# AuCson/DSP-Speech-Recognition

Measured on AMD Instinct MI355X. Metric: MFCC frames/sec at 16 kHz, 25 ms/10 ms, nfft=512, 40 mel, 13 cep, higher is better.
Workload: dtype f32; 1 GPU; configs[1]: batch of 1024 synthetic 1 s 16 kHz utterances -> MFCC+delta+delta2 [1024*99, 39] per step per GPU; frames_per_utterance=99, delta_n=2, input_buffers_rotated=8, hip_streams=3

## Files before the change

### dsp-speech-recognition_amd/csrc/kernels_fast512.h

```cpp
#pragma once

#include <cmath>
#include <cstdlib>
#include <type_traits>
#include <vector>

#include "dsp_common.h"
#include "launch_common.h"
#include "fft_inreg.h"

#define F512_WAVE_FLOATS 2112
#define F512_PS_STRIDE 264
#define F512_MAX_NI 6
#ifndef F512_WAVES
#define F512_WAVES 8
#endif
#ifndef F512_MIN_WAVES_PER_SIMD
#define F512_MIN_WAVES_PER_SIMD 4
#endif

struct F512Params {
    const float* tables;
    int32_t tab_floats;
    int32_t off_tw1, off_dct, off_melw, off_mels, off_bias, off_coop;
    int32_t melw_row;
    int32_t L, S, M, C, append_energy;
    float preemph;
    int32_t span_vec;
    int32_t nb4[F512_MAX_NI];
    int64_t groups_per_utt, total_groups;
    uint32_t t_magic, t_shift;
    uint32_t g_magic, g_shift;
    int32_t fd_n;
    float fd_inv_den;
    int32_t flat;
    int32_t seam_off;
    const int32_t* group_off;
    const int32_t* group_utt;
};

struct Fast512Plan {
    float* d_tables;
    F512Params P;
    int variant;
    int caps;
};

template <int CTRL>
__device__ __forceinline__ float dpp_f32(float v) {
    return __int_as_float(__builtin_amdgcn_update_dpp(0, __float_as_int(v), CTRL, 0xF, 0xF, true));
}
__device__ __forceinline__ float frame_allreduce(float v) {
    v += dpp_f32<0xB1>(v);
    v += dpp_f32<0x4E>(v);
    v += dpp_f32<0x141>(v);
    return v;
}

__host__ __device__ constexpr int f512_cap(int caps, int i) {
    constexpr int c1[5] = {2, 3, 4, 5, 8}, c2[4] = {3, 4, 6, 12};
    return caps == 1 ? c1[i] : c2[i];
}
__host__ __device__ constexpr int f512_cap_prefix(int caps, int i) {
    int s = 0;
    for (int k = 0; k < i; ++k) s += f512_cap(caps, k);
    return s;
}
template <int I, int N, typename F>
__device__ __forceinline__ void f512_static_for(F&& f) {
    if constexpr (I < N) {
        f(std::integral_constant<int, I>{});
        f512_static_for<I + 1, N>(f);
    }
}
__host__ __device__ constexpr int f512_cbase(int c) { return ((c & 1) ? 2 : 0) ^ ((c & 2) ? 4 : 0) ^ ((c & 4) ? 14 : 0); }
typedef float f512_f2u __attribute__((ext_vector_type(2), aligned(4)));

#define F512_FENCE() asm volatile("" ::: "memory")

#ifdef F512_STAMPS
#define F512_NSTAMP 16
__device__ unsigned int f512_stamp_sum[F512_NSTAMP * 8192];
__device__ __forceinline__ unsigned int f512_clock() {
    unsigned long long t;
    asm volatile("s_waitcnt lgkmcnt(0)\n\ts_memtime %0\n\ts_waitcnt lgkmcnt(0)" : "=s"(t) :: "memory");
    return (unsigned int)t;
}
template <typename T, int N>
__device__ __forceinline__ void f512_pin(T (&a)[N]) {
#pragma unroll
    for (int i = 0; i < N; ++i) {
        if constexpr (sizeof(T) == 8) asm volatile("" : "+v"(a[i].x), "+v"(a[i].y));
        else asm volatile("" : "+v"(a[i]));
    }
}
#ifdef F512_STAMP_ROUNDS
#define F512_STAMP(i)                                                         \
    do {                                                                      \
        if ((i) == 0) stamp_prev_ = f512_clock();                             \
        if ((i) == 10) {                                                      \
            stamp_acc_[r < 4 ? r : 3] += f512_clock() - stamp_prev_;          \
            stamp_acc_[4 + (r < 4 ? r : 3)] += 1;                             \
        }                                                                     \
    } while (0)
#else
#define F512_STAMP(i)                                     \
    do {                                                  \
        const unsigned int now_ = f512_clock();           \
        stamp_acc_[i] += now_ - stamp_prev_;              \
        stamp_prev_ = f512_clock();                       \
    } while (0)
#endif
#define F512_PIN(a) f512_pin(a)
#else
#define F512_STAMP(i) do {} while (0)
#define F512_PIN(a) do {} while (0)
#endif

typedef float f512_v2 __attribute__((ext_vector_type(2)));
__device__ __forceinline__ uint32_t f512_lds_addr(const void* p) {
    return static_cast<uint32_t>(reinterpret_cast<uintptr_t>(p));
}

template <int ROW0>
__device__ __forceinline__ void f512_load_rows8(uint32_t fr, uint32_t wn, f512_v2 (&xv)[8], f512_v2 (&wv)[8]) {
    asm volatile(
        "ds_read_b64 %0, %16 offset:%18\n\tds_read_b64 %8, %17 offset:%18\n\t"
        "ds_read_b64 %1, %16 offset:%19\n\tds_read_b64 %9, %17 offset:%19\n\t"
        "ds_read_b64 %2, %16 offset:%20\n\tds_read_b64 %10, %17 offset:%20\n\t"
        "ds_read_b64 %3, %16 offset:%21\n\tds_read_b64 %11, %17 offset:%21\n\t"
        "ds_read_b64 %4, %16 offset:%22\n\tds_read_b64 %12, %17 offset:%22\n\t"
        "ds_read_b64 %5, %16 offset:%23\n\tds_read_b64 %13, %17 offset:%23\n\t"
        "ds_read_b64 %6, %16 offset:%24\n\tds_read_b64 %14, %17 offset:%24\n\t"
        "ds_read_b64 %7, %16 offset:%25\n\tds_read_b64 %15, %17 offset:%25\n\t"
        "s_waitcnt lgkmcnt(0)"
        : "=&v"(xv[0]), "=&v"(xv[1]), "=&v"(xv[2]), "=&v"(xv[3]), "=&v"(xv[4]), "=&v"(xv[5]), "=&v"(xv[6]), "=&v"(xv[7]),
          "=&v"(wv[0]), "=&v"(wv[1]), "=&v"(wv[2]), "=&v"(wv[3]), "=&v"(wv[4]), "=&v"(wv[5]), "=&v"(wv[6]), "=&v"(wv[7])
        : "v"(fr), "v"(wn), "n"(64 * (ROW0 + 0)), "n"(64 * (ROW0 + 1)), "n"(64 * (ROW0 + 2)), "n"(64 * (ROW0 + 3)),
          "n"(64 * (ROW0 + 4)), "n"(64 * (ROW0 + 5)), "n"(64 * (ROW0 + 6)), "n"(64 * (ROW0 + 7))
        : "memory");
}
template <int ROW0>
__device__ __forceinline__ void f512_load_rows1(uint32_t fr, uint32_t wn, f512_v2& xv, f512_v2& wv) {
    asm volatile("ds_read_b64 %0, %2 offset:%4\n\tds_read_b64 %1, %3 offset:%4\n\ts_waitcnt lgkmcnt(0)"
                 : "=&v"(xv), "=&v"(wv) : "v"(fr), "v"(wn), "n"(64 * ROW0) : "memory");
}
template <int NROWS, int ROW0>
__device__ __forceinline__ void f512_window_rows(uint32_t fr, uint32_t wn, cpx (&z)[32]) {
    if constexpr (ROW0 + 8 <= NROWS) {
        f512_v2 xv[8], wv[8];
        f512_load_rows8<ROW0>(fr, wn, xv, wv);
#pragma unroll
        for (int r = 0; r < 8; ++r) z[ROW0 + r] = {xv[r].x * wv[r].x, xv[r].y * wv[r].y};
        f512_window_rows<NROWS, ROW0 + 8>(fr, wn, z);
    } else if constexpr (ROW0 < NROWS) {
        f512_v2 xv, wv;
        f512_load_rows1<ROW0>(fr, wn, xv, wv);
        z[ROW0] = {xv.x * wv.x, xv.y * wv.y};
        f512_window_rows<NROWS, ROW0 + 1>(fr, wn, z);
    }
}

template <int DTYPE> struct F512Raw { float4 v; };
template <> struct F512Raw<DSP_WAVE_I16> { short4 v; };

template <int DTYPE>
__device__ __forceinline__ F512Raw<DTYPE> f512_load_raw(const void* __restrict__ wave, int64_t idx) {
    F512Raw<DTYPE> r;
    if constexpr (DTYPE == DSP_WAVE_I16) r.v = *reinterpret_cast<const short4*>(reinterpret_cast<const int16_t*>(wave) + idx);
    else r.v = *reinterpret_cast<const float4*>(reinterpret_cast<const float*>(wave) + idx);
    return r;
}
typedef float f512_f4u __attribute__((ext_vector_type(4), aligned(4)));
typedef short f512_s4u __attribute__((ext_vector_type(4), aligned(2)));
template <int DTYPE>
__device__ __forceinline__ F512Raw<DTYPE> f512_load_raw_unaligned(const void* __restrict__ wave, int64_t idx) {
    F512Raw<DTYPE> r;
    if constexpr (DTYPE == DSP_WAVE_I16) {
        const f512_s4u t = *reinterpret_cast<const f512_s4u*>(reinterpret_cast<const int16_t*>(wave) + idx);
        r.v = make_short4(t.x, t.y, t.z, t.w);
    } else {
        const f512_f4u t = *reinterpret_cast<const f512_f4u*>(reinterpret_cast<const float*>(wave) + idx);
        r.v = make_float4(t.x, t.y, t.z, t.w);
    }
    return r;
}
template <int DTYPE>
__device__ __forceinline__ void f512_unpack(const F512Raw<DTYPE>& r, float (&x)[4]) {
    x[0] = (float)r.v.x; x[1] = (float)r.v.y; x[2] = (float)r.v.z; x[3] = (float)r.v.w;
}
__device__ __forceinline__ float f512_shift_in(float v, float left) {
    return __int_as_float(__builtin_amdgcn_update_dpp(__float_as_int(left), __float_as_int(v), 0x138, 0xF, 0xF, false));
}

static inline void f512_magic(uint32_t d, uint32_t& magic, uint32_t& shift) {
    uint32_t l = 0;
    while ((1ull << l) < d) ++l;
    shift = 30 + l;
    magic = (uint32_t)(((1ull << shift) + d - 1) / d);
}
__device__ __forceinline__ int f512_div(int x, uint32_t magic, uint32_t shift) {
    return (int)(((uint64_t)(uint32_t)x * magic) >> shift);
}

struct F512Group {
    int utt, t0, T, nsamp;
    int nf1;
    int64_t s0, row0;
};

template <bool RAGGED>
__device__ __forceinline__ F512Group f512_locate(const F512Params& P, const BatchGeom& bg, int G) {
    F512Group g;
    if constexpr (RAGGED) {
        g.utt = P.group_utt[G];
        g.t0 = (G - P.group_off[g.utt]) * 8;
        g.s0 = bg.sample_off[g.utt];
        g.nsamp = (int)(bg.sample_off[g.utt + 1] - g.s0);
        if (bg.seg != nullptr) {
            const int64_t lo = bg.seg[2 * g.utt];
            g.nsamp = (int)(bg.seg[2 * g.utt + 1] - lo);
            g.s0 += lo;
        }
        g.row0 = bg.frame_off[g.utt];
        g.T = (int)(bg.frame_off[g.utt + 1] - g.row0);
        g.nf1 = 8;
    } else {
        g.nsamp = (int)bg.uniform_samples;
        g.T = (int)bg.uniform_frames;
        if (P.flat) {
            const int F0 = 8 * G;
// ... 410 lines not shown
        cpx ra[16], rb[16];
#pragma unroll
        for (int k1 = 1; k1 < 16; ++k1) {
            const cpx zk = z[k1], zm = z[32 - k1];
            const cpx a = {zk.x + zm.x, zk.y - zm.y};
            const cpx b = {zk.y + zm.y, zm.x - zk.x};
            const float4 t = s_tw1[(k1 - 1) * 8 + c];
            ra[k1] = cmulc(a, t.x, t.y);
            rb[k1] = cmulc(b, t.z, t.w);
        }
#ifndef F512_COOP
        const float qa = 2.f * z[0].x, qb = 2.f * z[0].y, pa = 2.f * z[16].x, pb = 2.f * z[16].y;
#endif

        F512_PIN(ra); F512_PIN(rb);
        F512_STAMP(3);
        F512_PIN(ra); F512_PIN(rb);
        float* xb = wbuf + f * 256;
        cpx u0[16], u1[16];
        {
#ifndef F512_COOP
            const int s0x = sigma_hi;
            *reinterpret_cast<float2*>(xb + 4 * ((c >> 1) ^ s0x) + 2 * (c & 1)) = make_float2(qa + pa, qb + pb);
            *reinterpret_cast<float2*>(xb + 4 * ((4 + (c >> 1)) ^ s0x) + 2 * (c & 1)) = make_float2(qa - pa, qb - pb);
#endif
#pragma unroll
            for (int k1 = 1; k1 < 8; ++k1) {
                const int sg = (k1 >> 1) ^ sigma_hi;
                *reinterpret_cast<float4*>(xb + k1 * 32 + 4 * (np ^ sg)) = make_float4(ra[k1].x, ra[k1].y, rb[k1].x, rb[k1].y);
            }
            F512_FENCE();
            const int sg = (c >> 1) ^ sigma_hi;
#pragma unroll
            for (int i = 0; i < 8; ++i) {
                const float4 t = *reinterpret_cast<const float4*>(xb + c * 32 + 4 * (i ^ sg));
                u0[2 * i] = {t.x, t.y};
                u0[2 * i + 1] = {t.z, t.w};
            }
            F512_FENCE();
#pragma unroll
            for (int k1 = 8; k1 < 16; ++k1) {
                const int u = k1 - 8;
                const int sw = (u >> 1) ^ sigma_hi;
                *reinterpret_cast<float4*>(xb + u * 32 + 4 * (np ^ sw)) = make_float4(ra[k1].x, ra[k1].y, rb[k1].x, rb[k1].y);
            }
            F512_FENCE();
#pragma unroll
            for (int i = 0; i < 8; ++i) {
                const float4 t = *reinterpret_cast<const float4*>(xb + c * 32 + 4 * (i ^ sg));
                u1[2 * i] = {t.x, t.y};
                u1[2 * i + 1] = {t.z, t.w};
            }
            F512_FENCE();
        }

        F512_PIN(u0); F512_PIN(u1);
        F512_STAMP(4);
        F512_PIN(u0); F512_PIN(u1);
        FFTReg<16>::run(u0);
        FFTReg<16>::run(u1);
        F512_PIN(u0); F512_PIN(u1);
        F512_STAMP(5);
        F512_PIN(u0); F512_PIN(u1);

        float p0[16], p1[16];
        constexpr float S1 = 1.0f / 2048.0f;
#ifndef F512_COOP
        constexpr float S2 = 1.0f / 16.0f;
#endif
#pragma unroll
        for (int k = 0; k < 16; ++k) {
            p0[k] = fmaf(u0[k].x, u0[k].x, u0[k].y * u0[k].y);
            p1[k] = fmaf(u1[k].x, u1[k].x, u1[k].y * u1[k].y);
        }
#ifdef F512_COOP
        float e0 = p0[0], e1 = p1[0];
#pragma unroll
        for (int k = 1; k < 16; ++k) { e0 += p0[k]; e1 += p1[k]; }
        e0 = c == 0 ? coop_e8 : e0;
        e0 += coop_e + coop_o;
#else
        float podd[8];
        float e0 = p0[0], e1 = p1[0];
#pragma unroll
        for (int k = 1; k < 16; ++k) { e0 += p0[k]; e1 += p1[k]; }
#pragma unroll
        for (int m = 0; m < 8; ++m) podd[m] = 0.f;
        if (c == 0) {
            float R[17];
            const float f0 = u0[0].x + u0[0].y, f16 = u0[0].x - u0[0].y;
            R[0] = S2 * 4.f * f0 * f0;
            R[16] = S2 * 4.f * f16 * f16;
            R[8] = S2 * 4.f * fmaf(u0[8].x, u0[8].x, u0[8].y * u0[8].y);
#pragma unroll
            for (int j = 1; j < 8; ++j) {
                const cpx zj = u0[j], zq = u0[16 - j];
                const cpx e = {zj.x + zq.x, zj.y - zq.y};
                const cpx d = {zj.x - zq.x, zj.y + zq.y};
                const cpx o = {d.y, -d.x};
                const cpx tw = cmulc(o, DSP_COS32[j], -DSP_SIN32[j]);
                const cpx rp = {e.x + tw.x, e.y + tw.y};
                const cpx rm = {e.x - tw.x, e.y - tw.y};
                R[j] = S2 * fmaf(rp.x, rp.x, rp.y * rp.y);
                R[16 - j] = S2 * fmaf(rm.x, rm.x, rm.y * rm.y);
            }
            float es = R[0];
#pragma unroll
            for (int j = 1; j < 17; ++j) es += R[j];
            e0 = es;
#pragma unroll
            for (int k = 0; k < 8; ++k) {
                p0[k] = R[2 * k];
                p0[8 + k] = R[16 - 2 * k];
                podd[k] = R[2 * k + 1];
            }
        }
#endif
        float energy = (S1 * 4294967296.0f) * frame_allreduce(e0 + e1);

        F512_PIN(p0); F512_PIN(p1);
        F512_STAMP(6);
        F512_PIN(p0); F512_PIN(p1);
        float* ps = wbuf + f * F512_PS_STRIDE;
        {
            float* lo = ps + c;
            float* hi = ps + 32 - c;
#pragma unroll
            for (int k = 0; k < 8; ++k) {
                lo[32 * k] = p0[k];
                hi[32 * (7 - k)] = p0[8 + k];
                lo[32 * k + 8] = p1[k];
                hi[32 * (7 - k) - 8] = p1[8 + k];
            }
#ifdef F512_COOP
            F512_FENCE();
            ps[32 * coop_k] = coop_e;
            ps[32 * coop_k + 16] = coop_o;
            ps[256 + c] = c == 0 ? coop_e8 : 0.f;
#else
            if (c == 0) {
#pragma unroll
                for (int m = 0; m < 8; ++m) ps[32 * m + 16] = podd[m];
            } else {
                ps[256 + c] = 0.f;
            }
#endif
        }
        F512_FENCE();
        F512_STAMP(7);

        float lm[NI];
        {
            const float4* wrow = reinterpret_cast<const float4*>(s_melw + c * P.melw_row);
            f512_static_for<0, NI>([&](auto ic) {
                constexpr int i = decltype(ic)::value;
                const float4* pb = reinterpret_cast<const float4*>(ps + __float_as_int(smem[P.off_mels + i * 8 + c]));
                float acc0 = 0.f, acc1 = 0.f;
                if constexpr (CAPS != 0) {
                    constexpr int nb = f512_cap(CAPS, i), w0 = f512_cap_prefix(CAPS, i);
#pragma unroll
                    for (int b = 0; b < nb; ++b) {
                        const float4 w = wrow[w0 + b], q = pb[b];
                        acc0 = fmaf(w.x, q.x, acc0);
                        acc1 = fmaf(w.y, q.y, acc1);
                        acc0 = fmaf(w.z, q.z, acc0);
                        acc1 = fmaf(w.w, q.w, acc1);
                    }
                } else {
                    const int nb = P.nb4[i];
#pragma unroll 2
                    for (int b = 0; b < nb; ++b) {
                        const float4 w = wrow[b], q = pb[b];
                        acc0 = fmaf(w.x, q.x, acc0);
                        acc1 = fmaf(w.y, q.y, acc1);
                        acc0 = fmaf(w.z, q.z, acc0);
                        acc1 = fmaf(w.w, q.w, acc1);
                    }
                    wrow += nb;
                }
                const float acc = acc0 + acc1;
                const float l2 = __builtin_amdgcn_logf(acc);
                lm[i] = acc == 0.f ? -20.f : l2;
            });
        }
        F512_FENCE();
        F512_PIN(lm);
        F512_STAMP(8);
        F512_PIN(lm);

        float cep[16];
#pragma unroll
        for (int k = 0; k < 16; ++k) cep[k] = 0.f;
        constexpr int NU = (NI + 1) / 2;
#pragma unroll
        for (int u = 0; u < NU; ++u) {
            const float a = lm[u], b = dpp_f32<0x141>(lm[NI - 1 - u]);
            const float sm = a + b, df = a - b;
            const float4* dr = reinterpret_cast<const float4*>(s_dct + (u * 8 + c) * 20);
#pragma unroll
            for (int q = 0; q < 4; ++q) {
                const float4 t = dr[q];
                cep[4 * q + 0] = fmaf(t.x, sm, cep[4 * q + 0]);
                cep[4 * q + 1] = fmaf(t.y, df, cep[4 * q + 1]);
                cep[4 * q + 2] = fmaf(t.z, sm, cep[4 * q + 2]);
                cep[4 * q + 3] = fmaf(t.w, df, cep[4 * q + 3]);
            }
        }
        float h8[8], h4[4];
#pragma unroll
        for (int r = 0; r < 8; ++r) h8[r] = cep[r] + dpp_f32<0x141>(cep[8 + r]);
#pragma unroll
        for (int r = 0; r < 4; ++r) h4[r] = h8[r] + dpp_f32<0x4E>(h8[4 + r]);
        v0 = h4[0] + dpp_f32<0xB1>(h4[2]);
        v1 = h4[1] + dpp_f32<0xB1>(h4[3]);
        {
            const float2 bias = *reinterpret_cast<const float2*>(smem + P.off_bias + 2 * c);
            v0 += bias.x;
            v1 += bias.y;
        }
        if (P.append_energy) {
            constexpr float LN2 = 0.69314718055994530942f, LN_EPS = -36.04365338911715f;
            const float le = fmaf(__builtin_amdgcn_logf(energy), LN2, -32.f * LN2);
            if (c == 0) v0 = energy == 0.f ? LN_EPS : le;
        }

        F512_STAMP(9);
        if constexpr (!FD) {
            const int cb = ((c & 1) << 1) ^ ((c & 2) << 1) ^ ((c & 4) ? 14 : 0);
            const int t = t0 + f;
            const bool row_ok = (!RAGGED && P.flat) ? (grp.row0 + t < bg.total_frames) : (t < T);
            if (row_ok) {
                float* o = out + (grp.row0 + t) * ld_out + cb;
                if (cb + 1 < P.C) {
                    f512_f2u v;
                    v.x = v0;
                    v.y = v1;
                    *reinterpret_cast<f512_f2u*>(o) = v;
                } else if (cb < P.C) {
                    o[0] = v0;
                }
            }
        }
        } while (0);
        if constexpr (FD) {
            const int pr = (((c & 1) << 1) ^ ((c & 2) << 1) ^ ((c & 4) ? 14 : 0)) >> 1;
            const bool tail = r >= run.n_groups;
            if (r == 0) {
                if (pr < 7) *reinterpret_cast<float2*>(fd_halo + (wid * 8 + f) * 14 + 2 * pr) = make_float2(v0, v1);
                __syncthreads();
            }
            if (tail) {
                const int nw = wid + 1 < WAVES ? wid + 1 : wid;
                const float2 hv = *reinterpret_cast<const float2*>(fd_halo + (nw * 8 + f) * 14 + 2 * (pr < 7 ? pr : 0));
                v0 = hv.x;
                v1 = hv.y;
            }
            const bool emit = r > 0 || run.first_frame == run.wg_first;
            if (emit) {
                float* const tx = wbuf;
                float* const td = wbuf + 256;
                *reinterpret_cast<float2*>(tx + f * 16 + 2 * pr) = make_float2(fd_p0, fd_p1);
                *reinterpret_cast<float2*>(tx + (8 + f) * 16 + 2 * pr) = make_float2(v0, v1);
                const int Fw = run.first_frame + 8 * (r - 1);
                const int Tn = (int)bg.uniform_frames;
                const int tstart = (Fw + Tn) - f512_div(Fw + Tn, P.t_magic, P.t_shift) * Tn;
                const int sb = tstart == 0 ? 0 : Tn - tstart;
                constexpr int N = FD;
                const float inv_den = P.fd_inv_den;
                const int C = P.C;
                const int Fi = Fw + 4 + f;
                float* const o = out + (int64_t)Fi * (3 * C) + 2 * pr;
                float2 ox, od, odd;
                bool row_ok;
                F512_FENCE();
                if ((sb == 0 || sb >= 16) && Fw + 4 >= run.wg_first && Fw + 12 <= run.wg_end) {
                    const float* b = tx + f * 16 + 2 * pr;
                    float2 xr[4 * N + 1];
#pragma unroll
                    for (int k = 0; k <= 4 * N; ++k) xr[k] = *reinterpret_cast<const float2*>(b + (4 - 2 * N + k) * 16);
                    float2 dl[2 * N + 1];
#pragma unroll
                    for (int k = 0; k <= 2 * N; ++k) {
                        float a0 = 0.f, a1 = 0.f;
#pragma unroll
                        for (int n = 1; n <= N; ++n) {
                            a0 = fmaf((float)n, xr[N + k + n].x - xr[N + k - n].x, a0);
                            a1 = fmaf((float)n, xr[N + k + n].y - xr[N + k - n].y, a1);
                        }
                        dl[k] = make_float2(a0 * inv_den, a1 * inv_den);
                        asm volatile("" : "+v"(dl[k].x), "+v"(dl[k].y));
                    }
                    float a0 = 0.f, a1 = 0.f;
#pragma unroll
                    for (int n = 1; n <= N; ++n) {
                        a0 = fmaf((float)n, dl[N + n].x - dl[N - n].x, a0);
                        a1 = fmaf((float)n, dl[N + n].y - dl[N - n].y, a1);
                    }
                    ox = xr[2 * N];
                    od = dl[N];
                    odd = make_float2(a0 * inv_den, a1 * inv_den);
                    row_ok = true;
                } else {
#pragma unroll
                    for (int pass = 0; pass < 2; ++pass) {
                        const int i = pass == 0 ? 2 + f : (10 + f < 13 ? 10 + f : 13);
                        const int lo = i >= sb ? sb : 0, hi = i < sb ? sb - 1 : 15;
                        float a0 = 0.f, a1 = 0.f;
#pragma unroll
                        for (int n = 1; n <= N; ++n) {
                            const int ip = i + n < hi ? i + n : hi, im = i - n > lo ? i - n : lo;
                            const float2 xp = *reinterpret_cast<const float2*>(tx + ip * 16 + 2 * pr);
                            const float2 xm = *reinterpret_cast<const float2*>(tx + im * 16 + 2 * pr);
                            a0 = fmaf((float)n, xp.x - xm.x, a0);
                            a1 = fmaf((float)n, xp.y - xm.y, a1);
                        }
                        *reinterpret_cast<float2*>(td + i * 16 + 2 * pr) = make_float2(a0 * inv_den, a1 * inv_den);
                    }
                    F512_FENCE();
                    const int i = 4 + f;
                    const int lo = i >= sb ? sb : 0, hi = i < sb ? sb - 1 : 15;
                    float a0 = 0.f, a1 = 0.f;
#pragma unroll
                    for (int n = 1; n <= N; ++n) {
                        const int ip = i + n < hi ? i + n : hi, im = i - n > lo ? i - n : lo;
                        const float2 dp = *reinterpret_cast<const float2*>(td + ip * 16 + 2 * pr);
                        const float2 dm = *reinterpret_cast<const float2*>(td + im * 16 + 2 * pr);
                        a0 = fmaf((float)n, dp.x - dm.x, a0);
                        a1 = fmaf((float)n, dp.y - dm.y, a1);
                    }
                    ox = *reinterpret_cast<const float2*>(tx + i * 16 + 2 * pr);
                    od = *reinterpret_cast<const float2*>(td + i * 16 + 2 * pr);
                    odd = make_float2(a0 * inv_den, a1 * inv_den);
                    row_ok = Fi >= run.wg_first && Fi < run.wg_end;
                }
                if (row_ok) {
                    if (2 * pr + 1 < C) {
                        f512_f2u v;
                        v.x = ox.x; v.y = ox.y;
                        *reinterpret_cast<f512_f2u*>(o) = v;
                        v.x = od.x; v.y = od.y;
                        *reinterpret_cast<f512_f2u*>(o + C) = v;
                        v.x = odd.x; v.y = odd.y;
                        *reinterpret_cast<f512_f2u*>(o + 2 * C) = v;
                    } else if (2 * pr < C) {
                        o[0] = ox.x;
                        o[C] = od.x;
                        o[2 * C] = odd.x;
                    }
                }
            }
            fd_p0 = v0;
            fd_p1 = v1;
        }
        F512_FENCE();
        F512_STAMP(10);
    }
#ifdef F512_STAMPS
    stamp_acc_[11] = f512_clock() - stamp_entry_;
    stamp_acc_[12] = (unsigned int)__builtin_amdgcn_s_memrealtime() - stamp_rt0_;
    stamp_acc_[13] = stamp_loop0_ - stamp_entry_;
    stamp_acc_[14] = 1;
    if ((tid & 63) == 0) {
        const int slot = ((int)blockIdx.x * WAVES + wid) & 8191;
        for (int i = 0; i < F512_NSTAMP; ++i) f512_stamp_sum[slot * F512_NSTAMP + i] += stamp_acc_[i];
    }
#endif
}

static inline bool fast512_shape_ok(const dsp_plan_desc* d) {
    return d->nfft == 512 && d->frame_len <= 512 && (d->frame_step % 2) == 0 && d->frame_step >= 2 &&
           7 * d->frame_step + 512 + 16 <= F512_WAVE_FLOATS && d->nfilt >= 1 &&
           d->nfilt <= 8 * F512_MAX_NI && d->numcep >= 1 && d->numcep <= 16;
}

static inline bool fast512_dct_is_mirror_symmetric(const dsp_plan_desc* d) {
    const int M = d->nfilt, C = d->numcep;
    for (int k = 0; k < C; ++k) {
        double mx = 0.0;
        for (int j = 0; j < M; ++j) mx = std::max(mx, (double)std::fabs(d->h_dct[(size_t)k * M + j]));
        const double sgn = (k & 1) ? -1.0 : 1.0;
        for (int j = 0; j < M; ++j)
            if (std::fabs((double)d->h_dct[(size_t)k * M + (M - 1 - j)] - sgn * (double)d->h_dct[(size_t)k * M + j]) > 2e-6 * mx) return false;
    }
    return true;
}

static inline int fast512_plan_init(dsp_plan* p, const dsp_plan_desc* d, const int32_t* mel_off) {
    p->d_fast = nullptr;
    if (!fast512_shape_ok(d) || !d->h_dct || !fast512_dct_is_mirror_symmetric(d)) return DSP_OK;
    const int M = d->nfilt, C = d->numcep, L = d->frame_len;
    const int ni_real = (M + 7) / 8, nrows = (L + 15) / 16;
    int variant, NI;
    const int span25 = 7 * d->frame_step + 400, span32 = 7 * d->frame_step + 512;
    const int nstage = ((span25 + 3) / 4 + 1 + 63) / 64;
    if (nrows <= 25 && ni_real <= 4 && nstage <= 6) { variant = 0; NI = 4; }
    else if (nrows <= 25 && ni_real <= 5 && nstage <= 6) { variant = 1; NI = 5; }
    else { variant = 2; NI = F512_MAX_NI; }
    std::vector<float> win(512, 0.f);
    for (int n = 0; n < L; ++n) win[n] = d->h_window[n];
#ifdef F512_COOP
    auto col_pair = [](int c) { return c < 4 ? c : 11 - c; };
#else
    auto col_pair = [](int c) { return c; };
#endif
    std::vector<float> tw1(15 * 8 * 4);
    for (int k1 = 1; k1 < 16; ++k1)
        for (int c = 0; c < 8; ++c)
            for (int h = 0; h < 2; ++h) {
                const double a = -2.0 * M_PI * (double)((2 * col_pair(c) + h) * k1) / 512.0;
                tw1[((k1 - 1) * 8 + c) * 4 + 2 * h] = (float)cos(a);
                tw1[((k1 - 1) * 8 + c) * 4 + 2 * h + 1] = (float)sin(a);
            }
    std::vector<float> coop(8 * 16, 0.f);
    for (int c = 0; c < 8; ++c) {
        const int n = col_pair(c), n2 = n >> 2, n1 = (n >> 1) & 1, n0 = n & 1;
        const int k = n0 * 4 + n1 * 2 + n2;
        float* t = &coop[(size_t)c * 16];
        t[0] = n2 ? -1.f : 1.f;
        t[1] = n1 ? -1.f : 1.f;
        t[2] = n0 ? -1.f : 1.f;
        const double a1 = 2.0 * M_PI * (double)(n & 3) / 8.0, a2 = 2.0 * M_PI * (double)n0 / 4.0;
        t[4] = n2 ? (float)cos(a1) : 1.f;  t[5] = n2 ? (float)-sin(a1) : 0.f;
        t[6] = n1 ? (float)cos(a2) : 1.f;  t[7] = n1 ? (float)-sin(a2) : 0.f;
        const double ap = 2.0 * M_PI * (double)n / 16.0, ae = 2.0 * M_PI * (double)k / 16.0,
                     ao = 2.0 * M_PI * (double)(2 * k + 1) / 32.0;
        t[8] = (float)cos(ap);   t[9] = (float)-sin(ap);
        t[10] = (float)-sin(ae); t[11] = (float)-cos(ae);
        t[12] = (float)-sin(ao); t[13] = (float)-cos(ao);
        memcpy(&t[14], &k, 4);
    }
    std::vector<int> slot((size_t)8 * NI, -1);
    const int n_pairs = (M + 1) / 2, full = NI / 2;
    if (n_pairs > 4 * NI) return DSP_OK;
    for (int pr = 0; pr < n_pairs; ++pr) {
        const int ja = pr, jb = M - 1 - pr;
        int c, u;
        if (pr < 8 * full) { c = pr % 8; u = pr / 8; }
        else { c = pr - 8 * full; u = full; }
        slot[(size_t)u * 8 + c] = ja;
        slot[(size_t)(NI - 1 - u) * 8 + (7 - c)] = jb;
    }
    const int NU = (NI + 1) / 2;
    const double LN2 = 0.69314718055994530942;
    std::vector<float> dct((size_t)NU * 8 * 20, 0.f);
    std::vector<double> bias_acc(16, 0.0);
    for (int u = 0; u < NU; ++u)
        for (int c = 0; c < 8; ++c) {
            const int ja = slot[(size_t)u * 8 + c], jb = slot[(size_t)(NI - 1 - u) * 8 + (7 - c)];
            if (ja < 0) continue;
            const bool both = (NI & 1) && u == NI / 2;
            const double wgt = (both ? 0.5 : 1.0) * (ja == jb ? 0.5 : 1.0);
            for (int r = 0; r < 16; ++r) {
                const int k = r ^ f512_cbase(c);
                if (k >= C) continue;
                const float t = (float)(wgt * LN2 * (double)d->h_dct[(size_t)k * M + ja]);
                dct[((size_t)u * 8 + c) * 20 + r] = t;
                if ((r & 1) == 0) bias_acc[k] -= 64.0 * (double)t;
            }
        }
    std::vector<float> bias(16, 0.f);
    for (int c = 0; c < 8; ++c)
        for (int r = 0; r < 2; ++r) bias[2 * c + r] = (float)bias_acc[f512_cbase(c) + r];
    Fast512Plan* fp = new Fast512Plan();
    memset(fp, 0, sizeof(*fp));
    int caps = variant == 0 ? 2 : (variant == 1 ? 1 : 0);
    int row_blocks = 0;
    for (int i = 0; i < NI; ++i) {
        int len = 0;
        for (int c = 0; c < 8; ++c) {
            const int j = slot[(size_t)i * 8 + c];
            if (j < 0) continue;
            const int need = (d->h_mel_start[j] & 3) + d->h_mel_count[j];
            if (need > len) len = need;
        }
        fp->P.nb4[i] = (len + 3) / 4;
        if (caps != 0 && fp->P.nb4[i] > f512_cap(caps, i)) caps = 0;
    }
    for (int i = 0; i < NI; ++i) {
        if (caps != 0) fp->P.nb4[i] = f512_cap(caps, i);
        row_blocks += fp->P.nb4[i];
    }
    int melw_row = row_blocks > 0 ? 4 * row_blocks : 4;
    if (((melw_row / 4) & 1) == 0) melw_row += 4;
    std::vector<float> melw((size_t)8 * melw_row, 0.f), mels((size_t)NI * 8, 0.f);
    for (int c = 0; c < 8; ++c) {
        int pos = 0;
        for (int i = 0; i < NI; ++i) {
            const int j = slot[(size_t)i * 8 + c], len = 4 * fp->P.nb4[i];
            int32_t start = 0;
            if (j >= 0) {
                start = d->h_mel_start[j] & ~3;
                int lead = d->h_mel_start[j] - start;
                if (start + len > F512_PS_STRIDE) {
                    const int shift = (start + len - F512_PS_STRIDE + 3) / 4 * 4;
                    start -= shift;
                    lead += shift;
                }
                for (int s2 = 0; s2 < d->h_mel_count[j]; ++s2)
                    melw[(size_t)c * melw_row + pos + lead + s2] = d->h_mel_weights[mel_off[j] + s2] * 2097152.0f;
            }
            memcpy(&mels[(size_t)i * 8 + c], &start, 4);
            pos += len;
        }
    }
    auto pad64 = [](size_t n) { return (n + 63) / 64 * 64; };
    const size_t o_tw1 = 512, o_dct = o_tw1 + tw1.size(), o_melw = pad64(o_dct + dct.size());
    const size_t o_mels = o_melw + melw.size(), o_bias = o_mels + mels.size();
    const size_t o_coop = (o_bias + bias.size() + 3) / 4 * 4;
    const size_t total = pad64(o_coop + coop.size());
    std::vector<float> blob(total, 0.f);
    memcpy(blob.data(), win.data(), 512 * 4);
    memcpy(blob.data() + o_tw1, tw1.data(), tw1.size() * 4);
    memcpy(blob.data() + o_dct, dct.data(), dct.size() * 4);
    memcpy(blob.data() + o_melw, melw.data(), melw.size() * 4);
    memcpy(blob.data() + o_mels, mels.data(), mels.size() * 4);
    memcpy(blob.data() + o_bias, bias.data(), bias.size() * 4);
    memcpy(blob.data() + o_coop, coop.data(), coop.size() * 4);
    if (dsp_table_alloc_copy(reinterpret_cast<void**>(&fp->d_tables), blob.data(), total * 4) != hipSuccess) {
        delete fp;
        return DSP_EHIP;
    }
    fp->P.tables = fp->d_tables;
    fp->P.tab_floats = (int32_t)total;
    fp->P.off_tw1 = (int32_t)o_tw1; fp->P.off_dct = (int32_t)o_dct;
    fp->P.off_melw = (int32_t)o_melw; fp->P.off_mels = (int32_t)o_mels; fp->P.off_bias = (int32_t)o_bias;
    fp->P.off_coop = (int32_t)o_coop;
    fp->P.melw_row = melw_row;
    fp->P.L = L; fp->P.S = d->frame_step; fp->P.M = M; fp->P.C = C;
    fp->P.append_energy = d->append_energy ? 1 : 0;
    fp->P.preemph = d->preemph;
    fp->P.span_vec = ((variant == 2 ? span32 : span25) + 3) / 4;
    fp->variant = variant;
    fp->caps = caps;
    p->d_fast = fp;
    return DSP_OK;
}

static inline void fast512_plan_free(dsp_plan* p) {
    Fast512Plan* fp = static_cast<Fast512Plan*>(p->d_fast);
    if (!fp) return;
    dsp_table_free(fp->d_tables, p->dry_run);
    delete fp;
    p->d_fast = nullptr;
}

template <int NROWS, int NI, int CAPS, int NSTAGE, int DTYPE, bool RAGGED>
static int fast512_launch_k(const F512Params& P, const void* d_wave, const BatchGeom& bg, float* d_out,
                            int64_t ld_out, int64_t groups_bound, hipStream_t st) {
    const size_t lds = ((size_t)P.tab_floats + (size_t)F512_WAVES * F512_WAVE_FLOATS) * sizeof(float);
    const int64_t cap = (int64_t)dsp_cu_count() * (16 / F512_WAVES);
    int64_t blocks = (groups_bound + F512_WAVES - 1) / F512_WAVES;
    if (blocks > cap) blocks = cap;
    auto k = mfcc512_kernel<NROWS, NI, CAPS, NSTAGE, DTYPE, F512_WAVES, RAGGED>;
    static size_t granted[DSP_MAX_DEVICES] = {};
    if (dsp_ensure_dynamic_lds((const void*)k, lds, granted) != 0) return DSP_EHIP;
    k<<<(int)blocks, 64 * F512_WAVES, lds, st>>>(P, bg, d_wave, d_out, ld_out);
    return hipGetLastError() == hipSuccess ? DSP_OK : DSP_EHIP;
}

template <int NROWS, int NI, int CAPS, int NSTAGE>
static int fast512_launch_t(F512Params P, const void* d_wave, int dtype, const BatchGeom& bg, float* d_out,
                            int64_t ld_out, hipStream_t st, const DspRaggedTables* pre = nullptr) {
    if (bg.uniform_samples > 0) {
        P.groups_per_utt = (bg.uniform_frames + 7) / 8;
        P.total_groups = P.groups_per_utt * bg.n_utt;
        f512_magic((uint32_t)bg.uniform_frames, P.t_magic, P.t_shift);
        f512_magic((uint32_t)P.groups_per_utt, P.g_magic, P.g_shift);
        const int seam = (16 * NROWS - P.S + 3) / 4 * 4;
        if ((P.S % 4) == 0 && P.L > P.S && 16 * NROWS > P.S && bg.uniform_frames >= 8 && (bg.uniform_frames % 8) != 0 &&
            7 * P.S + 16 * NROWS + seam + 4 <= F512_WAVE_FLOATS && 7 * P.S + 16 * NROWS + seam <= 256 * (NSTAGE + 1) &&
            bg.total_frames + 8 <= 0x3fffffff) {
            P.flat = 1;
            P.seam_off = seam;
            P.total_groups = (bg.total_frames + 7) / 8;
        }
        return dsp_dispatch_wave(dtype, [&](auto dt) {
            return fast512_launch_k<NROWS, NI, CAPS, NSTAGE, decltype(dt)::value, false>(P, d_wave, bg, d_out, ld_out, P.total_groups, st);
        });
    }
    const int64_t bound = bg.total_frames / 8 + bg.n_utt;
    DspWorkspace* w;
    if (!dsp_ragged_tables_acquire(P, pre, 3, bg, bound, st, w)) return DSP_EHIP;
    const int rc = dsp_dispatch_wave(dtype, [&](auto dt) {
        return fast512_launch_k<NROWS, NI, CAPS, NSTAGE, decltype(dt)::value, true>(P, d_wave, bg, d_out, ld_out, bound, st);
    });
    return dsp_ragged_tables_release(w, st, rc);
}

static inline int fast512_launch(const dsp_plan* p, const void* d_wave, int dtype, const BatchGeom& bg,
                                 float* d_out, int64_t ld_out, hipStream_t st, const DspRaggedTables* pre = nullptr) {
    const Fast512Plan* fp = static_cast<const Fast512Plan*>(p->d_fast);
    if (fp->variant == 0 && fp->caps == 2) return fast512_launch_t<25, 4, 2, 6>(fp->P, d_wave, dtype, bg, d_out, ld_out, st, pre);
    if (fp->variant == 0) return fast512_launch_t<25, 4, 0, 6>(fp->P, d_wave, dtype, bg, d_out, ld_out, st, pre);
    if (fp->variant == 1 && fp->caps == 1) return fast512_launch_t<25, 5, 1, 6>(fp->P, d_wave, dtype, bg, d_out, ld_out, st, pre);
    if (fp->variant == 1) return fast512_launch_t<25, 5, 0, 6>(fp->P, d_wave, dtype, bg, d_out, ld_out, st, pre);
    return fast512_launch_t<32, F512_MAX_NI, 0, 9>(fp->P, d_wave, dtype, bg, d_out, ld_out, st, pre);
}

#define F512_FD_HALO_FLOATS (F512_WAVES * 8 * 14)

template <int NROWS, int NI, int CAPS, int NSTAGE>
static int fast512_launch_fused_t(F512Params P, const void* d_wave, int dtype, const BatchGeom& bg, int delta_n,
                                  float* d_out, hipStream_t st) {
    const int64_t T = bg.uniform_frames;
    const int64_t blocks = (int64_t)dsp_cu_count() * (16 / F512_WAVES);
    if (delta_n < 1 || delta_n > 2 || P.C > 14 || T < 8 * F512_WAVES - 7 || bg.n_utt < blocks) return 1;
    if ((P.S % 4) != 0 || P.L <= P.S || 16 * NROWS <= P.S) return 1;
    const int seam = (16 * NROWS - P.S + 3) / 4 * 4;
    if (7 * P.S + 16 * NROWS + seam + 4 > F512_WAVE_FLOATS || 7 * P.S + 16 * NROWS + seam > 256 * (NSTAGE + 1)) return 1;
    if (bg.total_frames + T + 16 > 0x3fffffff) return 1;
    P.flat = 1;
    P.seam_off = seam;
    P.groups_per_utt = (T + 7) / 8;
    P.total_groups = (bg.total_frames + 7) / 8;
    f512_magic((uint32_t)T, P.t_magic, P.t_shift);
    f512_magic((uint32_t)P.groups_per_utt, P.g_magic, P.g_shift);
    P.fd_n = delta_n;
    P.fd_inv_den = dsp_delta_inv_den(delta_n);
    const size_t lds = ((size_t)P.tab_floats + (size_t)F512_WAVES * F512_WAVE_FLOATS + F512_FD_HALO_FLOATS) * sizeof(float);
    if (lds > 80 * 1024) return 1;
    const int64_t ld = 3 * (int64_t)P.C;
    const int nblk = (int)blocks;
#define F512_FD_LAUNCH(DT, FDN)                                                                          \
    do {                                                                                                 \
        auto k = mfcc512_kernel<NROWS, NI, CAPS, NSTAGE, DT, F512_WAVES, false, FDN>;                    \
        static size_t granted[DSP_MAX_DEVICES] = {};                                                     \
        if (dsp_ensure_dynamic_lds((const void*)k, lds, granted) != 0) return DSP_EHIP;                  \
        k<<<nblk, 64 * F512_WAVES, lds, st>>>(P, bg, d_wave, d_out, ld);                                 \
    } while (0)
    if (dtype == DSP_WAVE_I16) {
        if (delta_n == 1) F512_FD_LAUNCH(DSP_WAVE_I16, 1); else F512_FD_LAUNCH(DSP_WAVE_I16, 2);
    } else {
        if (delta_n == 1) F512_FD_LAUNCH(DSP_WAVE_F32, 1); else F512_FD_LAUNCH(DSP_WAVE_F32, 2);
    }
#undef F512_FD_LAUNCH
    return hipGetLastError() == hipSuccess ? DSP_OK : DSP_EHIP;
}

static inline int fast512_launch_fused(const dsp_plan* p, const void* d_wave, int dtype, const BatchGeom& bg, int delta_n,
                                       float* d_out, hipStream_t st) {
    if (bg.uniform_samples <= 0) return 1;
    const Fast512Plan* fp = static_cast<const Fast512Plan*>(p->d_fast);
    if (fp->variant == 0 && fp->caps == 2) return fast512_launch_fused_t<25, 4, 2, 6>(fp->P, d_wave, dtype, bg, delta_n, d_out, st);
    if (fp->variant == 0) return fast512_launch_fused_t<25, 4, 0, 6>(fp->P, d_wave, dtype, bg, delta_n, d_out, st);
    if (fp->variant == 1 && fp->caps == 1) return fast512_launch_fused_t<25, 5, 1, 6>(fp->P, d_wave, dtype, bg, delta_n, d_out, st);
    if (fp->variant == 1) return fast512_launch_fused_t<25, 5, 0, 6>(fp->P, d_wave, dtype, bg, delta_n, d_out, st);
    return fast512_launch_fused_t<32, F512_MAX_NI, 0, 9>(fp->P, d_wave, dtype, bg, delta_n, d_out, st);
}
```

Measured before the change: 2.754 billion frames/s.

## Compute triangular mel filterbank in one pass using partition-of-unity masks

```diff
diff --git a/dsp-speech-recognition_amd/csrc/kernels_fast512.h b/dsp-speech-recognition_amd/csrc/kernels_fast512.h
--- a/dsp-speech-recognition_amd/csrc/kernels_fast512.h
+++ b/dsp-speech-recognition_amd/csrc/kernels_fast512.h
@@ -1,6 +1,7 @@
 #pragma once
 
 #include <cmath>
+#include <cstddef>
 #include <cstdlib>
 #include <type_traits>
 #include <vector>
@@ -12,6 +13,7 @@
 #define F512_WAVE_FLOATS 2112
 #define F512_PS_STRIDE 264
 #define F512_MAX_NI 6
+#define F512_OP_TAPS 56
 #ifndef F512_WAVES
 #define F512_WAVES 8
 #endif
@@ -28,6 +30,7 @@
     float preemph;
     int32_t span_vec;
     int32_t nb4[F512_MAX_NI];
+    uint64_t smask[F512_OP_TAPS];
     int64_t groups_per_utt, total_groups;
     uint32_t t_magic, t_shift;
     uint32_t g_magic, g_shift;
@@ -46,6 +49,9 @@
     int caps;
 };
 
+static_assert(offsetof(F512Params, smask) % 8 == 0, "the kernel reads P.smask as 64-bit words of the kernel argument segment");
+typedef __attribute__((address_space(4))) uint64_t F512KernargMask;
+
 template <int CTRL>
 __device__ __forceinline__ float dpp_f32(float v) {
     return __int_as_float(__builtin_amdgcn_update_dpp(0, __float_as_int(v), CTRL, 0xF, 0xF, true));
@@ -58,8 +64,8 @@
 }
 
 __host__ __device__ constexpr int f512_cap(int caps, int i) {
-    constexpr int c1[5] = {2, 3, 4, 5, 8}, c2[4] = {3, 4, 6, 12};
-    return caps == 1 ? c1[i] : c2[i];
+    constexpr int c1[5] = {2, 3, 4, 5, 8}, c2[4] = {3, 4, 6, 12}, c3[5] = {1, 2, 3, 3, 5};
+    return caps == 1 ? c1[i] : (caps == 2 ? c2[i] : c3[i]);
 }
 __host__ __device__ constexpr int f512_cap_prefix(int caps, int i) {
     int s = 0;
@@ -77,6 +83,19 @@
 typedef float f512_f2u __attribute__((ext_vector_type(2), aligned(4)));
 
 #define F512_FENCE() asm volatile("" ::: "memory")
+
+__device__ __forceinline__ float f512_masked_add4(float acc, const float4& q, uint64_t m0, uint64_t m1, uint64_t m2, uint64_t m3) {
+    uint64_t saved;
+    asm("s_mov_b64 %1, exec\n\t"
+        "s_mov_b64 exec, %6\n\tv_add_f32 %0, %0, %2\n\t"
+        "s_mov_b64 exec, %7\n\tv_add_f32 %0, %0, %3\n\t"
+        "s_mov_b64 exec, %8\n\tv_add_f32 %0, %0, %4\n\t"
+        "s_mov_b64 exec, %9\n\tv_add_f32 %0, %0, %5\n\t"
+        "s_mov_b64 exec, %1"
+        : "+v"(acc), "=&s"(saved)
+        : "v"(q.x), "v"(q.y), "v"(q.z), "v"(q.w), "s"(m0), "s"(m1), "s"(m2), "s"(m3));
+    return acc;
+}
 
 #ifdef F512_STAMPS
 #define F512_NSTAMP 16
@@ -793,11 +812,51 @@
         float lm[NI];
         {
             const float4* wrow = reinterpret_cast<const float4*>(s_melw + c * P.melw_row);
+            float op_carry = 0.f;
+            (void)op_carry;
             f512_static_for<0, NI>([&](auto ic) {
                 constexpr int i = decltype(ic)::value;
                 const float4* pb = reinterpret_cast<const float4*>(ps + __float_as_int(smem[P.off_mels + i * 8 + c]));
                 float acc0 = 0.f, acc1 = 0.f;
-                if constexpr (CAPS != 0) {
+                if constexpr (CAPS == 3) {
+                    constexpr int nb = f512_cap(3, i), w0 = 1 + f512_cap_prefix(3, i);
+                    if constexpr (i == 0) {
+                        const float4 w = wrow[0];
+                        const float4 q = *reinterpret_cast<const float4*>(ps + __float_as_int(smem[P.off_mels + NI * 8 + c]));
+                        op_carry = fmaf(w.x, q.x, w.y * q.y) + fmaf(w.z, q.z, w.w * q.w);
+                    }
+                    const F512KernargMask* mk = (const F512KernargMask*)__builtin_amdgcn_kernarg_segment_ptr() +
+                                                offsetof(F512Params, smask) / 8 + 4 * (w0 - 1);
+                    asm volatile("" : "+s"(mk));
+#ifdef F512_OP_PIN
+                    uint64_t mreg[4 * nb];
+#pragma unroll
+                    for (int k = 0; k < 4 * nb; ++k) mreg[k] = mk[k];
+#pragma unroll
+                    for (int k = 0; k < 4 * nb; ++k) asm volatile("" :: "s"(mreg[k]));
+#define F512_MK(k) mreg[k]
+#else
+#define F512_MK(k) mk[k]
+#endif
+                    float sum = 0.f;
+#pragma unroll
+                    for (int b = 0; b < nb; ++b) {
+                        const float4 w = wrow[w0 + b], q = pb[b];
+                        acc0 = fmaf(w.x, q.x, acc0);
+                        acc1 = fmaf(w.y, q.y, acc1);
+                        acc0 = fmaf(w.z, q.z, acc0);
+                        acc1 = fmaf(w.w, q.w, acc1);
+                        sum = f512_masked_add4(sum, q, F512_MK(4 * b), F512_MK(4 * b + 1), F512_MK(4 * b + 2), F512_MK(4 * b + 3));
+                    }
+                    const float rsum = acc0 + acc1;
+                    const float fall = fmaf(sum, 2097152.0f, -rsum);
+                    const float left = dpp_f32<0x111>(rsum);
+                    const float acc = (c == 0 ? op_carry : left) + fall;
+                    if constexpr (i + 1 < NI) op_carry = dpp_f32<0x107>(rsum);
+                    const float l2 = __builtin_amdgcn_logf(acc);
+                    lm[i] = acc == 0.f ? -20.f : l2;
+                    return;
+                } else if constexpr (CAPS != 0) {
                     constexpr int nb = f512_cap(CAPS, i), w0 = f512_cap_prefix(CAPS, i);
 #pragma unroll
                     for (int b = 0; b < nb; ++b) {
@@ -1026,6 +1085,76 @@
     return true;
 }
 
+struct F512OnePass {
+    std::vector<float> melw, mels;
+    int melw_row;
+    uint64_t smask[F512_OP_TAPS];
+};
+static inline bool f512_onepass_tables(const dsp_plan_desc* d, const int32_t* mel_off, const std::vector<int>& slot, int NI,
+                                       F512OnePass& t) {
+    constexpr int K = 257, M = 40;
+    if (d->nfilt != M || NI != 5) return false;
+    for (int j = 0; j < M; ++j)
+        if (slot[(size_t)j] != j) return false;
+    std::vector<float> W((size_t)M * K, 0.f);
+    for (int j = 0; j < M; ++j) {
+        if (d->h_mel_start[j] < 0 || d->h_mel_count[j] < 0 || d->h_mel_start[j] + d->h_mel_count[j] > K) return false;
+        for (int s2 = 0; s2 < d->h_mel_count[j]; ++s2) W[(size_t)j * K + d->h_mel_start[j] + s2] = d->h_mel_weights[mel_off[j] + s2];
+    }
+    int pk[M + 1];
+    for (int j = 0; j < M; ++j) {
+        pk[j] = -1;
+        for (int k = 0; k < K && pk[j] < 0; ++k)
+            if (std::fabs(W[(size_t)j * K + k] - 1.f) <= 1e-6f) pk[j] = k;
+        if (pk[j] < 0 || (j > 0 && pk[j] <= pk[j - 1])) return false;
+    }
+    pk[M] = d->h_mel_start[M - 1] + d->h_mel_count[M - 1];
+    if (pk[M] <= pk[M - 1]) return false;
+    for (int k = 0, seg = -1; k < K; ++k) {
+        while (seg + 1 < M && k >= pk[seg + 1]) ++seg;
+        float sum = 0.f;
+        for (int j = 0; j < M; ++j) {
+            const float w = W[(size_t)j * K + k];
+            if (w < 0.f) return false;
+            if (j == seg || j == seg + 1) sum += w;
+            else if (w != 0.f) return false;
+        }
+        if (seg >= 0 && seg < M - 1 && std::fabs(sum - 1.f) > 1e-6f) return false;
+    }
+    int row_blocks = 1;
+    for (int i = 0; i < NI; ++i) row_blocks += f512_cap(3, i);
+    if (4 * (row_blocks - 1) != F512_OP_TAPS) return false;
+    t.melw_row = 4 * row_blocks;
+    t.melw.assign((size_t)8 * t.melw_row, 0.f);
+    t.mels.assign((size_t)(NI + 1) * 8, 0.f);
+    memset(t.smask, 0, sizeof(t.smask));
+    constexpr float SCALE = 2097152.0f;
+    {
+        const int a = d->h_mel_start[0], b = pk[0];
+        if (b > a) {
+            const int32_t start = a & ~3;
+            if (b - start > 4) return false;
+            for (int k = a; k < b; ++k) t.melw[(size_t)(k - start)] = W[k] * SCALE;
+            memcpy(&t.mels[(size_t)NI * 8], &start, 4);
+        }
+    }
+    for (int j = 0; j < M; ++j) {
+        const int c = j % 8, i = j / 8, a = pk[j], b = pk[j + 1], len = 4 * f512_cap(3, i);
+        int32_t start = a & ~3;
+        if (start + len > F512_PS_STRIDE) start = (F512_PS_STRIDE - len) & ~3;
+        const int lead = a - start;
+        if (start < 0 || lead + (b - a) > len) return false;
+        const int pos = 4 * (1 + f512_cap_prefix(3, i));
+        for (int k = a; k < b; ++k) {
+            const float w = j + 1 < M ? W[(size_t)(j + 1) * K + k] : 1.f - W[(size_t)j * K + k];
+            t.melw[(size_t)c * t.melw_row + pos + lead + (k - a)] = w * SCALE;
+            t.smask[pos - 4 + lead + (k - a)] |= 0x0101010101010101ull << c;
+        }
+        memcpy(&t.mels[(size_t)i * 8 + c], &start, 4);
+    }
+    return true;
+}
+
 static inline int fast512_plan_init(dsp_plan* p, const dsp_plan_desc* d, const int32_t* mel_off) {
     p->d_fast = nullptr;
     if (!fast512_shape_ok(d) || !d->h_dct || !fast512_dct_is_mirror_symmetric(d)) return DSP_OK;
@@ -1105,6 +1234,8 @@
     Fast512Plan* fp = new Fast512Plan();
     memset(fp, 0, sizeof(*fp));
     int caps = variant == 0 ? 2 : (variant == 1 ? 1 : 0);
+    F512OnePass onepass;
+    if (variant == 1 && f512_onepass_tables(d, mel_off, slot, NI, onepass)) caps = 3;
     int row_blocks = 0;
     for (int i = 0; i < NI; ++i) {
         int len = 0;
@@ -1115,16 +1246,16 @@
             if (need > len) len = need;
         }
         fp->P.nb4[i] = (len + 3) / 4;
-        if (caps != 0 && fp->P.nb4[i] > f512_cap(caps, i)) caps = 0;
+        if (caps != 0 && caps != 3 && fp->P.nb4[i] > f512_cap(caps, i)) caps = 0;
     }
     for (int i = 0; i < NI; ++i) {
-        if (caps != 0) fp->P.nb4[i] = f512_cap(caps, i);
+        if (caps != 0 && caps != 3) fp->P.nb4[i] = f512_cap(caps, i);
         row_blocks += fp->P.nb4[i];
     }
     int melw_row = row_blocks > 0 ? 4 * row_blocks : 4;
     if (((melw_row / 4) & 1) == 0) melw_row += 4;
     std::vector<float> melw((size_t)8 * melw_row, 0.f), mels((size_t)NI * 8, 0.f);
-    for (int c = 0; c < 8; ++c) {
+    for (int c = 0; c < 8 && caps != 3; ++c) {
         int pos = 0;
         for (int i = 0; i < NI; ++i) {
             const int j = slot[(size_t)i * 8 + c], len = 4 * fp->P.nb4[i];
@@ -1143,6 +1274,12 @@
             memcpy(&mels[(size_t)i * 8 + c], &start, 4);
             pos += len;
         }
+    }
+    if (caps == 3) {
+        melw_row = onepass.melw_row;
+        melw.swap(onepass.melw);
+        mels.swap(onepass.mels);
+        memcpy(fp->P.smask, onepass.smask, sizeof(fp->P.smask));
     }
     auto pad64 = [](size_t n) { return (n + 63) / 64 * 64; };
     const size_t o_tw1 = 512, o_dct = o_tw1 + tw1.size(), o_melw = pad64(o_dct + dct.size());
@@ -1233,6 +1370,7 @@
     const Fast512Plan* fp = static_cast<const Fast512Plan*>(p->d_fast);
     if (fp->variant == 0 && fp->caps == 2) return fast512_launch_t<25, 4, 2, 6>(fp->P, d_wave, dtype, bg, d_out, ld_out, st, pre);
     if (fp->variant == 0) return fast512_launch_t<25, 4, 0, 6>(fp->P, d_wave, dtype, bg, d_out, ld_out, st, pre);
+    if (fp->variant == 1 && fp->caps == 3) return fast512_launch_t<25, 5, 3, 6>(fp->P, d_wave, dtype, bg, d_out, ld_out, st, pre);
     if (fp->variant == 1 && fp->caps == 1) return fast512_launch_t<25, 5, 1, 6>(fp->P, d_wave, dtype, bg, d_out, ld_out, st, pre);
     if (fp->variant == 1) return fast512_launch_t<25, 5, 0, 6>(fp->P, d_wave, dtype, bg, d_out, ld_out, st, pre);
     return fast512_launch_t<32, F512_MAX_NI, 0, 9>(fp->P, d_wave, dtype, bg, d_out, ld_out, st, pre);
@@ -1284,6 +1422,7 @@
     const Fast512Plan* fp = static_cast<const Fast512Plan*>(p->d_fast);
     if (fp->variant == 0 && fp->caps == 2) return fast512_launch_fused_t<25, 4, 2, 6>(fp->P, d_wave, dtype, bg, delta_n, d_out, st);
     if (fp->variant == 0) return fast512_launch_fused_t<25, 4, 0, 6>(fp->P, d_wave, dtype, bg, delta_n, d_out, st);
+    if (fp->variant == 1 && fp->caps == 3) return fast512_launch_fused_t<25, 5, 3, 6>(fp->P, d_wave, dtype, bg, delta_n, d_out, st);
     if (fp->variant == 1 && fp->caps == 1) return fast512_launch_fused_t<25, 5, 1, 6>(fp->P, d_wave, dtype, bg, delta_n, d_out, st);
     if (fp->variant == 1) return fast512_launch_fused_t<25, 5, 0, 6>(fp->P, d_wave, dtype, bg, delta_n, d_out, st);
     return fast512_launch_fused_t<32, F512_MAX_NI, 0, 9>(fp->P, d_wave, dtype, bg, delta_n, d_out, st);
```

New measurement: 2.713 billion frames/s. -1.5%, worse.
